# pangeo-data/scikit-downscale

Measured on AMD Instinct MI355X. Metric: grid-cells downscaled/sec (fit+predict), 40yr daily series, higher is better.
Workload: dtype f64; 1 GPU; BcsdTemperature quantile mapping, 100000 cells x 14600 steps per GPU (BASELINE configs[1]); cells_per_gpu=100000, total_cells=100000, groups=12, device= (gfx950:sramecc+:xnack-)

## Files before the change

scikit-downscale_amd/csrc/sd_bcsd_fx.hip:

```cpp
#include "sd_bcsd_rs.h"
#include "sd_wave.h"
#include "sd_wsort.h"

#ifdef SD_PHASE_MARKS
#define SDPH(name) asm volatile("; SDPHASE " name)
#else
#define SDPH(name)
#endif

namespace sdfx {

using namespace sdw;

#ifdef SD_DEV
constexpr int kTraceWgs = 256, kTraceSlots = 16, kTraceStride = 449;
__device__ long long sd_fx_trace[kTraceWgs * kTraceSlots];
#define SDT(slot)                                                                                              \
    do {                                                                                                       \
        if (traced) tstamp[slot] = (long long)__builtin_amdgcn_s_memtime();                                    \
    } while (0)
#else
#define SDT(slot)
#endif
using sdrs::Params;
// ... 570 lines not shown
                double v[K];
#pragma unroll
                for (int i = 0; i < K; ++i) v[i] = ob[i];
                double s = 0.0;
                if constexpr (FULL) {
#pragma unroll
                    for (int i = 0; i < K; ++i) s += v[i];
                    s = K * lane < n ? s : 0.0;
                } else {
#pragma unroll
                    for (int i = 0; i < K; ++i) s += K * lane + i < n ? v[i] : 0.0;
                }
                yc = wave_sum_f64(s) / (double)n;
                make_keys<K, false, FULL>(v, n, lane, ky);
            }
            SDT(10);
            SDPH("y_sort");
            if (!(abl & 2)) sdws::wave_sort<K>(ky, lane, (n + K - 1) / K);
            SDT(11);
            SDPH("y_fix");
            if (!(abl & 8)) redo_y = (fix_equal_q<K>(ky, rowb, lane) & kUnsorted) != 0 && cell_live;
            SDPH("y_gather");
            if constexpr (FULL) {
                const unsigned tm = K * lane < n ? kTagMask : 0u;
#pragma unroll
                for (int i = 0; i < K; ++i) t[i] = lds_f64(rowb + 8u * (ky[i] & tm));
            } else {
#pragma unroll
                for (int i = 0; i < K; ++i) t[i] = lds_f64(rowb + 8u * (K * lane + i < n ? (ky[i] & kTagMask) : (unsigned)(RS - 1)));
            }
            if (!IDENT) {
                wave_fence();
#pragma unroll
                for (int i = 0; i < K; ++i) lds_store_f64(K * lane + i < n ? rowb + 8u * (unsigned)(K * lane + i) : spare, t[i]);
            }
        }
    } else {
        SD_LANE();
        if (cell_ok) {
            yc = p->y_climo[seg];
            const double* src = p->ys + c * p->Tf + begf;
            for (int i = lane; i < n; i += kWave) row[i] = src[i];
        }
        wave_fence();
        if (IDENT) {
            const double* srow = row + (K * lane < n ? K * lane : 0);
#pragma unroll
            for (int i = 0; i < K; ++i) t[i] = srow[i];
        }
    }

    SDT(12);
    SDPH("map_scatter");
    int to[NR];
    {
        SD_LANE();
        if (!IDENT) {
            wave_fence();
            double slo = 0.0, ilo = 0.0, shi = 0.0, ihi = 0.0;
            if (m > n && n > 0) {
                const int e = n < p->n_endpoints ? n : p->n_endpoints;
                const double dn = pp_denom(n);
                ols_line(row, 0, e, dn, &slo, &ilo);
                ols_line(row, n - e, e, dn, &shi, &ihi);
            }
            const double nan = __longlong_as_double(0x7ff8000000000000ll);
            const int r0 = K * lane < m ? K * lane : 0;
            const int32_t* qi = p->qidx + begp + r0;
            const double* qv = p->qval + begp + r0;
#pragma unroll
            for (int i = 0; i < K; ++i) {
                const bool in = r0 + i < m;
                const int idx = in ? qi[i] : -3;
                const double w = in ? qv[i] : 0.0;
                double v;
                if (idx >= 0) {
                    const double y0 = row[idx];
                    const double y1 = row[idx + 1 < n ? idx + 1 : idx];
                    v = w == 0.0 ? y0 : y0 + w * (y1 - y0);
                } else if (idx == -1) {
                    v = w * slo + ilo;
                } else if (idx == -2) {
                    v = w * shi + ihi;
                } else {
                    v = nan;
                }
                t[i] = v;
                if ((i + 1) % CH == 0) __builtin_amdgcn_sched_barrier(0);
            }
        }
        wave_fence();
        const bool has = K * lane < m;
        if constexpr (FULL) {
            if (has) {
#pragma unroll
                for (int i = 0; i < K; ++i) lds_store_f64(rowb + 8u * (ku[i] & kTagMask), t[i]);
            }
        } else {
#pragma unroll
            for (int i = 0; i < K; ++i) lds_store_f64(K * lane + i < m ? rowb + 8u * (ku[i] & kTagMask) : spare, t[i]);
        }
        wave_fence();
        SDPH("restore");
        if (kEarlyRows) rows_load<NR, FULL>(p->ord_p + begp, m, to);
        double* ob = row + L::own(has ? lane : 0);
        double q[K];
#pragma unroll
        for (int i = 0; i < K; ++i) q[i] = ob[i];
        const double ycr = p->return_anoms ? yc : 0.0;
        if constexpr (FULL) {
            if (has) {
#pragma unroll
                for (int i = 0; i < K; ++i) ob[i] = (shift[i] + q[i]) - ycr;
            }
        } else {
#pragma unroll
            for (int i = 0; i < K; ++i) {
                const double res = (shift[i] + q[i]) - ycr;
                lds_store_f64(K * lane + i < m ? rowb + 8u * (unsigned)(L::own(lane) + i) : spare, res);
            }
        }
    }
    SDPH("store");
    SDT(13);
    redo_flag[wave] = redo_y ? 1 : 0;
    __syncthreads();
    SDT(14);
    any_redo = 0;
#pragma unroll
    for (int w = 0; w < kW; ++w) any_redo |= redo_flag[w];
    if (any_redo) {
        if (threadIdx.x == 0) {
            const int slot = atomicAdd(p->work_count, 1);
            if (slot < p->work_cap) p->worklist[slot] = tile_id * p->G + g;
        }
        return;
    }
    const bool vec_o = (p->ld_out % 2 == 0) && ((reinterpret_cast<uintptr_t>(p->out) & 15) == 0);
        if (!kEarlyRows) rows_load<NR, FULL>(p->ord_p + begp, m, to);
    if (!(abl & 16)) store_tile_ti<K, FULL>(p->out, p->ld_out, to, m, c0, p->C, vec_o, tile, RS);
#ifdef SD_DEV
    SDT(15);
    if (traced && threadIdx.x == 0) {
#pragma unroll
        for (int i = 0; i < kTraceSlots; ++i) sd_fx_trace[(blockIdx.x / kTraceStride) * kTraceSlots + i] = tstamp[i];
    }
#endif
#undef SD_LANE
}

namespace tmj {
constexpr int kChunkStride = 1024 + 8;
constexpr int kBlock = 20;
__host__ __device__ constexpr int chunks_of(int n) { return n / kBlock + 16; }
__device__ __forceinline__ int tail_chunk(int l) { return (l & 7) + 8 * (l >> 5); }
__device__ __forceinline__ int tail_slot(int l) { return (l >> 3) & 3; }
__device__ __forceinline__ int row_of_slot(int Q, int S, int nl, int n) {
    int r;
    if (Q < nl) {
        r = kBlock * Q + S;
    } else {
        const int t = Q - nl;
        const int l = (t & 7) + 8 * (S & 3) + 32 * (t >> 3);
        r = l < nl ? kBlock * l + 16 + (S >> 2) : n - 1;
    }
    return r < n ? r : n - 1;
}
__device__ __forceinline__ unsigned tag_off(unsigned tag) { return (tag << 6) + ((tag >> 4) << 3); }

template <int NREG>
struct RowIdx {
    int v[NREG];
};
template <int NREG>
__device__ __forceinline__ RowIdx<NREG> rows_of_wave(const int32_t* __restrict__ ord, int n, int q0, int wave, int lane) {
    RowIdx<NREG> t;
    const int nl = n / kBlock;
#pragma unroll
    for (int j = 0; j < NREG; ++j) {
        const int e = 64 * j + lane;
        t.v[j] = ord[row_of_slot(q0 + wave + kW * (e >> 4), e & 15, nl, n)];
    }
    return t;
}
template <int NREG>
__device__ __forceinline__ void rows_ready(RowIdx<NREG>& t) {
#pragma unroll
    for (int j = 0; j < NREG; ++j) asm volatile("" : "+v"(t.v[j]));
}
template <int NREG>
__device__ __forceinline__ int row_of_request(const RowIdx<NREG>& rows, int k, int lane) {
    return __builtin_amdgcn_ds_bpermute(4 * (16 * (k & 3) + (lane >> 2)), rows.v[k >> 2]);
}
template <int NK, int NREG>
__device__ __forceinline__ void dma_chunks(const double* __restrict__ src, int64_t ld, const RowIdx<NREG>& rows, int q0, int q1,
                                           int64_t c0, unsigned tile_b, int wave, int lane) {
    static_assert(NK <= 4 * NREG, "row registers");
    const char* colp = reinterpret_cast<const char*>(src + c0) + 16 * (lane & 3);
#pragma unroll
    for (int k = 0; k < NK; ++k) {
        const int q = q0 + wave + kW * k;
        if (q < q1) {
            const int ti = row_of_request(rows, k, lane);
            const char* g = colp + (uint64_t)(uint32_t)ti * (uint64_t)(uint32_t)((uint32_t)ld * 8u);
            const int dst = __builtin_amdgcn_readfirstlane((int)(tile_b + (unsigned)q * (unsigned)kChunkStride));
            unsigned keep;
            asm volatile("s_mov_b32 %0, m0\n\ts_mov_b32 m0, %2\n\ts_nop 0\n\tglobal_load_lds_dwordx4 %1, off\n\ts_mov_b32 m0, %0"
                         : "=&s"(keep)
                         : "v"(g), "s"(dst)
                         : "memory");
        }
    }
}
__device__ __forceinline__ void dma_wait_all() { asm volatile("s_waitcnt vmcnt(0)" ::: "memory"); }

struct Col {
    unsigned mainb, tailb, prevb;
    __device__ __forceinline__ unsigned at(int idx) const {
        return idx < 0 ? prevb + (unsigned)(256 * (idx + 4)) : idx < 16 ? mainb + (unsigned)(64 * idx)
             : idx < 20 ? tailb + (unsigned)(256 * (idx - 16)) : mainb + (unsigned)(kChunkStride + 64 * (idx - 20));
    }
    __device__ __forceinline__ double get(int idx) const {
        if (idx < 0) return reinterpret_cast<lds_cdouble_t*>((uintptr_t)prevb)[32 * (idx + 4)];
        if (idx < 16) return reinterpret_cast<lds_cdouble_t*>((uintptr_t)mainb)[8 * idx];
        if (idx < 20) return reinterpret_cast<lds_cdouble_t*>((uintptr_t)tailb)[32 * (idx - 16)];
        return reinterpret_cast<lds_cdouble_t*>((uintptr_t)mainb)[kChunkStride / 8 + 8 * (idx - 20)];
    }
    __device__ __forceinline__ void put(int idx, double x) const {
        if (idx < 16) reinterpret_cast<lds_double_t*>((uintptr_t)mainb)[8 * idx] = x;
        else reinterpret_cast<lds_double_t*>((uintptr_t)tailb)[32 * (idx - 16)] = x;
    }
};
__device__ __forceinline__ Col col_of(unsigned tile_b, int col, int bl, int nl) {
    const unsigned cb = tile_b + 8u * (unsigned)col;
    const int lp = (bl - 1) & 63;
    Col c;
    c.mainb = cb + (unsigned)bl * (unsigned)kChunkStride;
    c.tailb = cb + (unsigned)(nl + tail_chunk(bl)) * (unsigned)kChunkStride + 64u * (unsigned)tail_slot(bl);
    c.prevb = cb + (unsigned)(nl + tail_chunk(lp)) * (unsigned)kChunkStride + 64u * (unsigned)tail_slot(lp);
    return c;
}
struct Tags {
    unsigned main0, tail0;
    __device__ __forceinline__ unsigned of(int i) const { return i < 16 ? main0 + (unsigned)i : tail0 + (unsigned)(4 * (i - 16)); }
};
__device__ __forceinline__ Tags tags_of(int lane, int nl) {
    return Tags{16u * (unsigned)lane, 16u * (unsigned)(nl + tail_chunk(lane)) + (unsigned)tail_slot(lane)};
}

template <int K, class GetU>
__device__ __forceinline__ void keys_u2(const GetU& u_of, double lo, double hi, int m, int lane, const Tags& tg, unsigned (&key)[K], unsigned (&u2)[K]) {
    const double sc = (double)(kQD - 2u) / (hi - lo);
    const double off = -lo * sc + 1.0;
    const unsigned tag0 = (unsigned)(K * lane);
    const unsigned pad0 = ((kQD + 1u + tag0) << kTagBits) | tag0;
    const bool lane_in = K * lane < m;
#pragma unroll
    for (int i = 0; i < K; ++i) {
        const double t = __builtin_fma(u_of(i), sc, off) + 2097152.0;
        const unsigned w0 = (unsigned)__double2loint(t), w1 = (unsigned)__double2hiint(t);
        unsigned q = __builtin_amdgcn_alignbit(w1, w0, 31) & 0x1fffffu;
        q = q < kQD ? q : kQD;
        const unsigned dk = (q << kTagBits) | tg.of(i);
        const unsigned pk = pad0 + (unsigned)i * ((1u << kTagBits) + 1u);
        key[i] = lane_in ? dk : pk;
        u2[i] = w0;
    }
}
template <int K>
__device__ __forceinline__ void keys_pos(const double (&v)[K], int m, int lane, const Tags& tg, unsigned (&key)[K]) {
    double lo = __builtin_inf(), hi = -__builtin_inf();
#pragma unroll
    for (int i = 0; i < K; ++i) {
        lo = vmin(lo, v[i]);
        hi = vmax(hi, v[i]);
    }
    lo = wave_min_f64(lo);
    hi = wave_max_f64(hi);
    const double sc = (double)kQD / (hi - lo);
    const double off = -lo * sc;
    const unsigned tag0 = (unsigned)(K * lane);
    const unsigned pad0 = ((kQD + 1u + tag0) << kTagBits) | tag0;
    const bool lane_in = K * lane < m;
#pragma unroll
    for (int i = 0; i < K; ++i) {
        unsigned q = (unsigned)__builtin_fma(v[i], sc, off);
        q = q < kQD ? q : kQD;
        const unsigned dk = (q << kTagBits) | tg.of(i);
        const unsigned pk = pad0 + (unsigned)i * ((1u << kTagBits) + 1u);
        key[i] = lane_in ? dk : pk;
    }
}

template <int K, class Cmp>
__device__ __forceinline__ int fix_equal_q_by(unsigned (&k)[K], int lane, const Cmp& cmp) {
    constexpr unsigned kQ = 1u << kTagBits;
    bool tie = false;
#pragma unroll 1
    for (int pass = 0; pass < 6; ++pass) {
        bool swapped = false;
        const unsigned knext = from_next_lane(k[0], 0xffffffffu);
        const bool eqx = (k[K - 1] ^ knext) < kQ;
        const unsigned long long bx = __ballot(eqx);
        if (bx != 0ull) {
            bool gt, eq;
            cmp(k[K - 1] & kTagMask, knext & kTagMask, &gt, &eq);
            const bool sw = eqx && gt;
            tie |= eqx && eq;
            const unsigned d = sw ? (k[K - 1] ^ knext) : 0u;
            k[K - 1] ^= d;
            k[0] ^= from_prev_lane(d, 0u);
            swapped |= sw;
        }
        unsigned long long prev = 0ull, b0 = 0ull, multi = 0ull;
#pragma unroll
        for (int i = 0; i + 1 < K; ++i) {
            const bool e = (k[i] ^ k[i + 1]) < kQ;
            const unsigned long long b = __ballot(e);
            multi |= b & prev;
            if (i == 0) b0 = b;
            prev = b;
            if (b != 0ull) {
                bool gt, eq;
                cmp(k[i] & kTagMask, k[i + 1] & kTagMask, &gt, &eq);
                const bool sw = e && gt;
                tie |= e && eq;
                const unsigned d = sw ? (k[i] ^ k[i + 1]) : 0u;
                k[i] ^= d;
                k[i + 1] ^= d;
                swapped |= sw;
            }
        }
        multi |= (bx & prev) | ((bx << 1) & b0);
        if (multi == 0ull || !__any(swapped)) return __any(tie) ? kTie : 0;
    }
    return kUnsorted;
}
}

__host__ __device__ constexpr int fd_u2_stride(int nmax) { return 16 * tmj::chunks_of(nmax); }
__host__ __device__ constexpr int fd_late_chunks(int rsu) { return (kW * 4 * rsu + tmj::kChunkStride - 1) / tmj::kChunkStride; }
inline size_t fd_lds_bytes(int nmax) { return (size_t)kHeadDoubles * sizeof(double) + (size_t)tmj::chunks_of(nmax) * tmj::kChunkStride; }

template <int K, bool EARLY>
__global__ void __launch_bounds__(kThreads, 4) bcsd_fd_kernel(const Params) {
    extern __shared__ __attribute__((aligned(16))) char smem_raw[];
    ParamsPtr p = (ParamsPtr)__builtin_amdgcn_kernarg_segment_ptr();
    constexpr int NR = K / 2;
    constexpr int CH = K >= 20 ? K / 4 : K >= 14 ? K / 2 : K;
    constexpr int NKX = 10;
    static_assert(K == tmj::kBlock && K % CH == 0, "the chunk layout is that of 20 rows per lane");
#ifdef SD_DEV
    const int abl = p->dev_flags;
#else
    constexpr int abl = 0;
#endif
    double* const scratch = reinterpret_cast<double*>(smem_raw);
    int* const bad_cell = reinterpret_cast<int*>(scratch + 64 + 16);
    int* const redo_flag = bad_cell + kW;
    const unsigned tile_b = lds_addr(smem_raw) + (unsigned)(kHeadDoubles * sizeof(double));
    if (threadIdx.x >= 32 && threadIdx.x < 32 + kW) bad_cell[threadIdx.x - 32] = 0;
#ifdef SD_DEV
    const bool traced = (abl & 0x800) != 0 && blockIdx.x % kTraceStride == 7 && blockIdx.x / kTraceStride < (unsigned)kTraceWgs;
    long long tstamp[kTraceSlots] = {};
    SDT(0);
#endif
    int64_t tile_id;
    int g;
    xcd_tile_of_block(blockIdx.x, p->ntiles, &tile_id, &g);
    if (p->gmask != 0ull) g = nth_set_bit(p->gmask, g);
    if (tile_id >= p->ntiles || g < 0 || g >= p->G) return;

    const int64_t c0 = tile_id * kW;
    const int wave = __builtin_amdgcn_readfirstlane(tid_now() / kWave);
#define SD_LANE() const int lane = tid_now() % kWave
    const int64_t c = c0 + wave;
    const bool cell_ok = c < p->C;
    const int begf = p->off_f[g];
    const int m = p->off_f[g + 1] - begf;
    const int begp = p->off_p[g];
    if (m == 0) return;
    const int nl = m / K;
    const int nch = tmj::chunks_of(m);
    const int RSU = p->RS;
    const int nlate = fd_late_chunks(RSU) < nch ? fd_late_chunks(RSU) : nch;
    const bool cell_live = cell_ok && p->status_fit[cell_ok ? c : 0] == 0;
    const int64_t cfetch = c0 + kW <= p->C ? c0 : p->C - kW;
    const int cshift = (int)(c0 - cfetch);
    const int col = wave + cshift < kW ? wave + cshift : wave + cshift - kW;
    __syncthreads();

    SDPH("x_tiles");
    double xc = 0.0;
    tmj::RowIdx<EARLY ? 2 : 3> ry_late;
    tmj::RowIdx<2> ry_early;
    {
        SD_LANE();
        tmj::RowIdx<3> rp = tmj::rows_of_wave<3>(p->ord_p + begp, m, 0, wave, lane);
        TileRegs<NR> xh;
        int tf[NR];
        rows_load<NR, true>(p->ord_f + begf, m, tf);
        tmj::rows_ready(rp);
#pragma unroll
        for (int k = 0; k < NR; ++k) asm volatile("" : "+v"(tf[k]));
        if (!(abl & 64)) tmj::dma_chunks<NKX, 3>(p->Xp, p->ld_p, rp, 0, nch, cfetch, tile_b, wave, lane);
        if (!(abl & 4)) {
            const int cp = lane & 3;
            const double* src = p->X + (c0 + 2 * cp + 1 < p->C ? c0 + 2 * cp : c0);
#pragma unroll
            for (int k = 0; k < NR; ++k) {
                const double2 v = *reinterpret_cast<const double2*>(row_of(src, tf[k], p->ld));
                xh.v0[k] = v.x;
                xh.v1[k] = v.y;
            }
        }
        if (!(abl & 4)) tile_reduce_partials<NR, true>(xh, m, c0, p->C, scratch, p->status_fit, wave, lane, bad_cell);
        SDT(1);
        tmj::dma_wait_all();
    }
    __syncthreads();
    SDT(2);
    {
        double tot = 0.0;
#pragma unroll
        for (int w = 0; w < kW; ++w) tot += scratch[w * kW + wave];
        xc = tot / (double)m;
    }

    SDPH("rolling");
    double shift[K];
    unsigned ku[K];
    bool redo = false;
    {
        SD_LANE();
        const bool has = K * lane < m;
        const int bl = has ? lane : 0;
        const bool first_lane = bl == 0, last_lane = K * (bl + 1) == m;
        const tmj::Col cz = tmj::col_of(tile_b, col, bl, nl);
        double ulo = __builtin_inf(), uhi = -__builtin_inf();
        bool bad = false;
#pragma unroll
        for (int cbeg = 0; cbeg < K; cbeg += CH) {
            double w[CH + 8];
#pragma unroll
            for (int t = 0; t < CH + 8; ++t) {
                const int idx = cbeg - 4 + t;
                const double x = cz.get(idx);
                w[t] = idx < 0 ? (first_lane ? 0.0 : x) : idx >= K ? (last_lane ? 0.0 : x) : x;
            }
#pragma unroll
            for (int ii = 0; ii < CH; ++ii) {
                double s = 0.0;
#pragma unroll
                for (int d = 0; d < 9; ++d) s += w[ii + d];
                const int i = cbeg + ii;
                constexpr double kRc[10] = {0.0, 1.0, 0.5, 1.0 / 3.0, 0.25, 0.2, 1.0 / 6.0, 1.0 / 7.0, 0.125, 1.0 / 9.0};
                double cd = 9.0, rc = kRc[9];
                if (i < 4) {
                    cd = first_lane ? (double)(5 + i) : cd;
                    rc = first_lane ? kRc[5 + i] : rc;
                }
                if (i >= K - 4) {
                    cd = last_lane ? (double)(K + 4 - i) : cd;
                    rc = last_lane ? kRc[K + 4 - i] : rc;
                }
                const double q = s * rc;
                const double mean = __builtin_fma(__builtin_fma(-cd, q, s), rc, q);
                const double sh = mean - xc;
                shift[i] = sh;
                bad |= nonfinite64(w[ii + 4]);
                const double ui = (w[ii + 4] - sh) + 0.0;
                ulo = vmin(ulo, ui);
                uhi = vmax(uhi, ui);
            }
            __builtin_amdgcn_sched_barrier(0);
        }
        if (__any(bad && has)) {
            if (lane == 0) {
                if (cell_ok) atomicOr(&p->status_p[c], SDI_NONFINITE);
                bad_cell[wave] = 1;
            }
        }
        SDT(3);
        ry_late = tmj::rows_of_wave<EARLY ? 2 : 3>(p->ord_f + begf, m, 0, wave, lane);
        if (EARLY) ry_early = tmj::rows_of_wave<2>(p->ord_f + begf, m, nlate, wave, lane);
        SDPH("u_keys");
        unsigned u2[K];
        {
            ulo = wave_min_f64(ulo);
            uhi = wave_max_f64(uhi);
            const auto u_of = [&](int i) { return (cz.get(i) - shift[i]) + 0.0; };
            tmj::keys_u2<K>(u_of, ulo, uhi, m, lane, tmj::tags_of(lane, nl), ku, u2);
        }
        tmj::rows_ready(ry_late);
        unsigned ub;
        if constexpr (EARLY) {
            tmj::rows_ready(ry_early);
            __syncthreads();
            if (!(abl & 32)) tmj::dma_chunks<5, 2>(p->y, p->ld, ry_early, nlate, nch, cfetch, tile_b, wave, lane);
            ub = tile_b + 4u * (unsigned)(col * RSU);
        } else {
            wave_fence();
            ub = 0u;
        }
        if (!EARLY) {
            if (has) {
                const tmj::Col cw = tmj::col_of(tile_b, col, lane, nl);
#pragma unroll
                for (int i = 0; i < K; ++i) *reinterpret_cast<__attribute__((address_space(3))) unsigned*>((uintptr_t)cw.at(i)) = u2[i];
            }
        } else if (has) {
            const tmj::Tags tg = tmj::tags_of(lane, nl);
            typedef unsigned __attribute__((ext_vector_type(4))) u32x4;
            __attribute__((address_space(3))) u32x4* um = reinterpret_cast<__attribute__((address_space(3))) u32x4*>((uintptr_t)(ub + 4u * tg.main0));
#pragma unroll
            for (int i = 0; i < 16; i += 4) um[i / 4] = u32x4{u2[i], u2[i + 1], u2[i + 2], u2[i + 3]};
            __attribute__((address_space(3))) unsigned* ut = reinterpret_cast<__attribute__((address_space(3))) unsigned*>((uintptr_t)(ub + 4u * tg.tail0));
#pragma unroll
            for (int i = 16; i < K; ++i) ut[4 * (i - 16)] = u2[i];
        }
        wave_fence();
        SDT(4);
        SDPH("u_sort");
        if (!(abl & 1)) sdws::wave_sort<K>(ku, lane, (m + K - 1) / K);
        SDT(5);
        SDPH("u_fix");
        const unsigned colb_u = tile_b + 8u * (unsigned)col;
        const auto cmp_u2 = [ub, colb_u](unsigned ta, unsigned tb, bool* gt, bool* eq) {
            const unsigned a = lds_u32(EARLY ? ub + 4u * ta : colb_u + tmj::tag_off(ta)), b = lds_u32(EARLY ? ub + 4u * tb : colb_u + tmj::tag_off(tb));
            *gt = a > b;
            *eq = a == b;
        };
        const bool tie = (abl & 8) ? false : tmj::fix_equal_q_by<K>(ku, lane, cmp_u2) != 0;
        redo = tie && cell_live && bad_cell[wave] == 0 && (abl & 0x7ff) == 0;
        SDT(6);
    }
    SDPH("vote");
    redo_flag[wave] = redo ? 1 : 0;
    __syncthreads();
    int any_redo = 0;
#pragma unroll
    for (int w = 0; w < kW; ++w) any_redo |= redo_flag[w];
    if (any_redo) {
        tmj::dma_wait_all();
        if (threadIdx.x == 0) {
            const int slot = atomicAdd(p->work_count, 1);
            if (slot < p->work_cap) p->worklist[slot] = tile_id * p->G + g;
        }
        return;
    }
    SDT(7);

    SDPH("y_tile");
    double yc = 0.0;
    double t[K];
    bool redo_y = false;
    {
        SD_LANE();
        if (!(abl & 32)) tmj::dma_chunks<EARLY ? 5 : NKX, EARLY ? 2 : 3>(p->y, p->ld, ry_late, 0, EARLY ? nlate : nch, cfetch, tile_b, wave, lane);
        SDT(8);
        tmj::dma_wait_all();
        __syncthreads();
        SDT(9);
        SDPH("y_keys");
        const bool has = K * lane < m;
        const int bl = has ? lane : 0;
        const tmj::Col cz = tmj::col_of(tile_b, col, bl, nl);
        const unsigned colb = tile_b + 8u * (unsigned)col;
        unsigned ky[K];
        {
            double v[K];
#pragma unroll
            for (int i = 0; i < K; ++i) v[i] = cz.get(i);
            double s = 0.0;
            bool bad = false;
#pragma unroll
            for (int i = 0; i < K; ++i) {
                s += v[i];
                bad |= nonfinite64(v[i]);
            }
            s = has ? s : 0.0;
            yc = wave_sum_f64(s) / (double)m;
            if (__any(bad && has) && lane == 0 && cell_ok) atomicOr(&p->status_fit[c], SDI_NONFINITE);
            tmj::keys_pos<K>(v, m, lane, tmj::tags_of(lane, nl), ky);
        }
        SDT(10);
        SDPH("y_sort");
        if (!(abl & 2)) sdws::wave_sort<K>(ky, lane, (m + K - 1) / K);
        SDT(11);
        SDPH("y_fix");
        const auto cmp_y = [colb](unsigned ta, unsigned tb, bool* gt, bool* eq) {
            const double a = lds_f64(colb + tmj::tag_off(ta)), b = lds_f64(colb + tmj::tag_off(tb));
            *gt = a > b;
            *eq = a == b;
        };
        if (!(abl & 8)) redo_y = (tmj::fix_equal_q_by<K>(ky, lane, cmp_y) & kUnsorted) != 0 && cell_live;
        SDPH("y_gather");
        {
            const unsigned tm = has ? kTagMask : 0u;
#pragma unroll
            for (int i = 0; i < K; ++i) t[i] = lds_f64(colb + tmj::tag_off(ky[i] & tm));
        }
        SDT(12);
        SDPH("map_scatter");
        wave_fence();
        if (has) {
#pragma unroll
            for (int i = 0; i < K; ++i) lds_store_f64(colb + tmj::tag_off(ku[i] & kTagMask), t[i]);
        }
        wave_fence();
        SDPH("restore");
        double q[K];
#pragma unroll
        for (int i = 0; i < K; ++i) q[i] = cz.get(i);
        const double ycr = p->return_anoms ? yc : 0.0;
        if (has) {
#pragma unroll
            for (int i = 0; i < K; ++i) cz.put(i, (shift[i] + q[i]) - ycr);
        }
    }
    SDPH("store");
    SDT(13);
    redo_flag[wave] = redo_y ? 1 : 0;
    tmj::RowIdx<3> ro = tmj::rows_of_wave<3>(p->ord_p + begp, m, 0, wave, tid_now() % kWave);
    __syncthreads();
    tmj::rows_ready(ro);
    SDT(14);
    any_redo = 0;
#pragma unroll
    for (int w = 0; w < kW; ++w) any_redo |= redo_flag[w];
    if (any_redo) {
        if (threadIdx.x == 0) {
            const int slot = atomicAdd(p->work_count, 1);
            if (slot < p->work_cap) p->worklist[slot] = tile_id * p->G + g;
        }
        return;
    }
    if (!(abl & 16)) {
        SD_LANE();
        const int pair = 2 * (lane & 3);
        const bool keep = pair >= cshift;
        char* colp = reinterpret_cast<char*>(p->out + cfetch) + 16 * (lane & 3);
#pragma unroll
        for (int k = 0; k < NKX; ++k) {
            const int qc = wave + kW * k;
            const int S = lane >> 2;
            const bool row_in = qc < nl ? K * qc + S < m : (((qc - nl) & 7) + 8 * (S & 3) + 32 * ((qc - nl) >> 3)) < nl;
            const int ti = tmj::row_of_request(ro, k, lane);
            if (qc < nch && row_in && keep) {
                typedef double __attribute__((ext_vector_type(2))) f64x2;
                const f64x2 v = *reinterpret_cast<__attribute__((address_space(3))) const f64x2*>((uintptr_t)(tile_b + (unsigned)qc * (unsigned)tmj::kChunkStride + 16u * (unsigned)lane));
                *reinterpret_cast<f64x2*>(colp + (uint64_t)(uint32_t)ti * (uint64_t)(uint32_t)((uint32_t)p->ld_out * 8u)) = v;
            }
        }
    }
#ifdef SD_DEV
    SDT(15);
    if (traced && threadIdx.x == 0) {
#pragma unroll
        for (int i = 0; i < kTraceSlots; ++i) sd_fx_trace[(blockIdx.x / kTraceStride) * kTraceSlots + i] = tstamp[i];
    }
#endif
#undef SD_LANE
}

template <int K, bool IDENT, bool FULL>
__device__ __forceinline__ void fxp_segment(ParamsPtr p, int64_t tile_id, int g, char* smem_raw) {
    static_assert(!FULL || IDENT, "FULL launches serve groups of equal fit / predict length");
    constexpr int NR = K / 2;
    constexpr int CH = K >= 20 ? K / 4 : K >= 14 ? K / 2 : K;
    using L = Lay<K>;
    double* const scratch = reinterpret_cast<double*>(smem_raw);
    int* const bad_cell = reinterpret_cast<int*>(scratch + 64 + 16);
    int* const redo_flag = bad_cell + kW;
    double* const tile = scratch + kHeadDoubles;
    const int RS = p->RS;
    if (threadIdx.x >= 32 && threadIdx.x < 32 + kW) bad_cell[threadIdx.x - 32] = 0;

    const int64_t c0 = tile_id * kW;
    const int wave = __builtin_amdgcn_readfirstlane(tid_now() / kWave);
#define SD_LANE() const int lane = tid_now() % kWave
    const int64_t c = c0 + wave;
    const bool cell_ok = c < p->C;
    double* const row = tile + wave * RS;
    const unsigned rowb = lds_addr(row);
    const int64_t seg = c * p->G + g;
    const int begf = p->off_f[g];
    const int n = p->off_f[g + 1] - begf;
    const int begp = p->off_p[g];
    const int m = p->off_p[g + 1] - begp;
    if (m == 0) return;
    const bool vec_f = (p->ld % 2 == 0) && ((reinterpret_cast<uintptr_t>(p->y) & 15) == 0) &&
                       (p->X == nullptr || (reinterpret_cast<uintptr_t>(p->X) & 15) == 0);
    const bool vec_p = (p->ld_p % 2 == 0) && ((reinterpret_cast<uintptr_t>(p->Xp) & 15) == 0);
    const bool cell_live = cell_ok && p->status_fit[cell_ok ? c : 0] == 0;
    const unsigned spare = rowb + 8u * (unsigned)(RS - 1);
    __syncthreads();

    {
        TileRegs<NR> xf;
        int tp[NR];
        rows_load<NR, FULL>(p->ord_p + begp, m, tp);
        if (!p->from_state && p->X != nullptr && n > 0) {
            TileRegs<NR> xh;
            int tf[NR];
            rows_load<NR, FULL>(p->ord_f + begf, n, tf);
            tile_issue_ti<NR>(p->X, p->ld, tf, c0, p->C, vec_f, xh);
            tile_issue_ti<NR>(p->Xp, p->ld_p, tp, c0, p->C, vec_p, xf);
            tile_check_finite<NR>(xh, n, c0, p->C, p->status_fit, bad_cell);
        } else {
            tile_issue_ti<NR>(p->Xp, p->ld_p, tp, c0, p->C, vec_p, xf);
        }
        tile_commit_sw<NR, K, FULL>(xf, m, c0, p->C, tile, RS, p->status_p, bad_cell);
    }
    __syncthreads();

    unsigned ku[K];
    int n0 = 0;
    bool redo = false;
    TileRegs<NR> yt;
    {
        SD_LANE();
        const double* ob = row + L::own(K * lane < m ? lane : 0);
        double v[K];
#pragma unroll
        for (int i = 0; i < K; ++i) v[i] = ob[i];
        if constexpr (FULL) {
            const bool has = K * lane < m;
#pragma unroll
            for (int i = 0; i < K; ++i) n0 += __popcll(__ballot(has && v[i] == 0.0));
        } else {
#pragma unroll
            for (int i = 0; i < K; ++i) n0 += __popcll(__ballot(K * lane + i < m && v[i] == 0.0));
        }
        const double lo = make_keys<K, true, FULL>(v, m, lane, ku);
        if (!p->from_state && n > 0) {
            int ty[NR];
            rows_load<NR, FULL>(p->ord_f + begf, n, ty);
            tile_issue_ti<NR>(p->y, p->ld, ty, c0, p->C, vec_f, yt);
        }
        sdws::wave_sort<K>(ku, lane, (m + K - 1) / K);
        const bool tie = fix_equal_q<K, true>(ku, rowb, lane) != 0;
        redo = (tie || lo < 0.0) && cell_live && bad_cell[wave] == 0;
    }
    redo_flag[wave] = redo ? 1 : 0;
    __syncthreads();
    int any_redo = 0;
#pragma unroll
    for (int w = 0; w < kW; ++w) any_redo |= redo_flag[w];
    if (any_redo) {
        if (threadIdx.x == 0) {
            const int slot = atomicAdd(p->work_count, 1);
            if (slot < p->work_cap) p->worklist[slot] = tile_id * p->G + g;
        }
        return;
    }

    double yc = 0.0;
    bool redo_y = false;
    if (!p->from_state) {
        if (n > 0) {
            SD_LANE();
            tile_commit_sw<NR, K, FULL>(yt, n, c0, p->C, tile, RS, p->status_fit, nullptr);
            __syncthreads();
            unsigned ky[K];
            {
                const double* ob = row + L::own(K * lane < n ? lane : 0);
                double v[K];
#pragma unroll
                for (int i = 0; i < K; ++i) v[i] = ob[i];
                double s = 0.0;
                if constexpr (FULL) {
#pragma unroll
                    for (int i = 0; i < K; ++i) s += v[i];
                    s = K * lane < n ? s : 0.0;
                } else {
#pragma unroll
                    for (int i = 0; i < K; ++i) s += K * lane + i < n ? v[i] : 0.0;
                }
                yc = wave_sum_f64(s) / (double)n;
                if (lane == 0 && cell_ok && p->return_anoms && yc <= 0.0) atomicOr(&p->status_fit[c], SDI_BAD_CLIMO);
                const double lo = make_keys<K, true, FULL>(v, n, lane, ky);
                redo_y = lo < 0.0 && cell_live;
            }
            sdws::wave_sort<K>(ky, lane, (n + K - 1) / K);
            redo_y = (redo_y || (fix_equal_q<K, true>(ky, rowb, lane) & kUnsorted) != 0) && cell_live;
            double t[K];
            if constexpr (FULL) {
                const unsigned tm = K * lane < n ? kTagMask : 0u;
#pragma unroll
                for (int i = 0; i < K; ++i) t[i] = lds_f64(rowb + 8u * (ky[i] & tm));
            } else {
#pragma unroll
                for (int i = 0; i < K; ++i) t[i] = lds_f64(rowb + 8u * (K * lane + i < n ? (ky[i] & kTagMask) : (unsigned)(RS - 1)));
            }
            wave_fence();
            if constexpr (FULL) {
                if (K * lane < n) {
#pragma unroll
                    for (int i = 0; i < K; ++i) lds_store_f64(rowb + 8u * (unsigned)(K * lane + i), t[i]);
// ... 306 lines not shown
            const double lo = make_keys_plain<KC>(vc, nw_y, lane, ky);
            sdws::wave_sort<KC>(ky, lane, (nw_y + KC - 1) / KC);
            redo_y = (lo < 0.0 || (fix_equal_q<KC>(ky, rowb, lane) & kUnsorted) != 0) && cell_live;
            double t[KC];
            const unsigned tm = KC * lane < nw_y ? kTagMask : 0u;
#pragma unroll
            for (int i = 0; i < KC; ++i) t[i] = lds_f64(rowb + 8u * (ky[i] & tm));
            wave_fence();
            if (KC * lane < nw_y) {
#pragma unroll
                for (int i = 0; i < KC; ++i) lds_store_f64(KC * lane + i < nw_y ? rowb + 8u * (unsigned)(KC * lane + i) : spare, t[i]);
            }
            wave_fence();
        }
    }

    int to[NR];
    {
        SD_LANE();
        const int n0_x = m - nw_x;
        auto ys = [&](int r) -> double {
            const double w = row[r >= n0_y ? r - n0_y : 0];
            return r >= n0_y ? w : 0.0;
        };
        double t[KC];
#pragma unroll
        for (int i = 0; i < KC; ++i) {
            const int rw = KC * lane + i;
            t[i] = ys(rw < nw_x ? n0_x + rw : 0);
        }
        const double val0 = ys(n0_x > 0 ? n0_x - 1 : 0);
        wave_fence();
        if (KC * lane < nw_x) {
#pragma unroll
            for (int i = 0; i < KC; ++i) lds_store_f64(KC * lane + i < nw_x ? rowb + 8u * (kx[i] & kTagMask) : spare, t[i]);
        }
        wave_fence();
        double q[K];
        {
            const double* cp = row + base_x;
            int pos = 0;
#pragma unroll
            for (int i = 0; i < K; ++i) {
                const bool wet = ((zm_x >> i) & 1u) == 0u;
                const double wv = cp[wet ? pos : 0];
                q[i] = wet ? wv : val0;
                pos += wet ? 1 : 0;
            }
        }
        wave_fence();
        const bool has = K * lane < m;
        rows_load<NR, FULL>(p->ord_p + begp, m, to);
        if (has) {
            double* ob = row + L::own(lane);
            const double rc = 1.0 / yc;
#pragma unroll
            for (int i = 0; i < K; ++i) {
                double res = q[i];
                if (p->return_anoms) {
                    const double a = q[i] * rc;
                    res = __builtin_fma(__builtin_fma(-yc, a, q[i]), rc, a);
                    res = __builtin_isfinite(res) ? res : q[i] / yc;
                }
                ob[i] = res;
            }
        }
    }
    redo_flag[wave] = (redo_y ? 1 : 0) | (many_y ? 2 : 0);
    __syncthreads();
    any_redo = 0;
#pragma unroll
    for (int w = 0; w < kW; ++w) any_redo |= redo_flag[w];
    if (any_redo) {
        if (threadIdx.x == 0) {
            if (any_redo & 1) {
                const int slot = atomicAdd(p->work_count, 1);
                if (slot < p->work_cap) p->worklist[slot] = tile_id * p->G + g;
            } else {
                const int slot = atomicAdd(p->work_count2, 1);
                if (slot < p->work_cap) p->worklist2[slot] = tile_id * p->G + g;
            }
        }
        return;
    }
    const bool vec_o = (p->ld_out % 2 == 0) && ((reinterpret_cast<uintptr_t>(p->out) & 15) == 0);
    store_tile_ti<K, FULL>(p->out, p->ld_out, to, m, c0, p->C, vec_o, tile, RS);
#undef SD_LANE
}

template <int K, bool IDENT, bool FULL>
int launch_one(sd_ctx* ctx, const Params& p, size_t lds) {
    const int64_t tx = (p.ntiles + 7) / 8;
    const int64_t nblocks = 8 * tx * (p.gmask ? __builtin_popcountll(p.gmask) : p.G);
    SD_CHECK_ARG(nblocks < ((int64_t)1 << 31), "grid too large");
    if (p.kind == SD_BCSD_TAS) {
        SD_HIP(hipFuncSetAttribute(reinterpret_cast<const void*>(&bcsd_fx_kernel<K, IDENT, FULL>), hipFuncAttributeMaxDynamicSharedMemorySize,
                                   (int)lds));
        SD_LAUNCH(ctx, FULL ? "bcsd_fx_kernel_full" : "bcsd_fx_kernel", (bcsd_fx_kernel<K, IDENT, FULL>), dim3((unsigned)nblocks),
                  dim3(kThreads), lds, p);
    } else {
        SD_HIP(hipFuncSetAttribute(reinterpret_cast<const void*>(&bcsd_fxp_kernel<K, IDENT, FULL>), hipFuncAttributeMaxDynamicSharedMemorySize,
                                   (int)lds));
        SD_LAUNCH(ctx, FULL ? "bcsd_fxp_kernel_full" : "bcsd_fxp_kernel", (bcsd_fxp_kernel<K, IDENT, FULL>), dim3((unsigned)nblocks),
                  dim3(kThreads), lds, p);
    }
    return SD_OK;
}

template <int K, bool IDENT>
int launch_ki(sd_ctx* ctx, Params p, int nmax, const int* group_len) {
    p.RS = row_slots<K>(nmax);
    const size_t lds = ((size_t)kW * p.RS + kHeadDoubles) * sizeof(double);
    if (lds > ctx->lds_max) return sd_set_error(SD_ERR_UNSUPPORTED, "segment of %d samples needs %zu bytes of LDS", nmax, lds);
    unsigned long long full = 0ull, rest = 0ull;
#ifndef SD_FX_NOFULL
    if (IDENT && group_len != nullptr && p.G <= 64 && sd_dev_env("SD_FX_NOFULL") == nullptr) {
        for (int g = 0; g < p.G; ++g) {
            const bool f = group_len[g] % K == 0 && group_len[g] >= full_min_len<K>();
            (f ? full : rest) |= 1ull << g;
        }
    }
#endif
#ifndef SD_FX_NOCOMPACT
    if constexpr (IDENT && compact_width<K>() != 0) {
        if (p.kind == SD_BCSD_PR && !p.from_state && p.work_count2 != nullptr && p.G <= 64 && group_len != nullptr &&
            sd_dev_env("SD_FX_NOCOMPACT") == nullptr) {
            constexpr int KC = compact_width<K>();
            Params q = p;
            if ((full | rest) == 0ull) rest = p.G == 64 ? ~0ull : (1ull << p.G) - 1ull;
            if (full != 0ull) {
                q.gmask = full;
                const int64_t nb = 8 * ((p.ntiles + 7) / 8) * __builtin_popcountll(full);
                SD_CHECK_ARG(nb < ((int64_t)1 << 31), "grid too large");
                SD_HIP(hipFuncSetAttribute(reinterpret_cast<const void*>(&bcsd_fxc_kernel<K, KC, true>), hipFuncAttributeMaxDynamicSharedMemorySize, (int)lds));
                SD_LAUNCH(ctx, "bcsd_fxc_kernel_full", (bcsd_fxc_kernel<K, KC, true>), dim3((unsigned)nb), dim3(kThreads), lds, q);
            }
            if (rest != 0ull) {
                q.gmask = rest;
                const int64_t nb = 8 * ((p.ntiles + 7) / 8) * __builtin_popcountll(rest);
                SD_CHECK_ARG(nb < ((int64_t)1 << 31), "grid too large");
                SD_HIP(hipFuncSetAttribute(reinterpret_cast<const void*>(&bcsd_fxc_kernel<K, KC, false>), hipFuncAttributeMaxDynamicSharedMemorySize, (int)lds));
                SD_LAUNCH(ctx, "bcsd_fxc_kernel", (bcsd_fxc_kernel<K, KC, false>), dim3((unsigned)nb), dim3(kThreads), lds, q);
            }
            Params r = p;
            r.use_worklist = 2;
            SD_HIP(hipFuncSetAttribute(reinterpret_cast<const void*>(&bcsd_fxp_kernel<K, IDENT, false>), hipFuncAttributeMaxDynamicSharedMemorySize, (int)lds));
            SD_LAUNCH(ctx, "bcsd_fxp_kernel_list", (bcsd_fxp_kernel<K, IDENT, false>), dim3((unsigned)(2 * (ctx->cu_count > 0 ? ctx->cu_count : 256))),
                      dim3(kThreads), lds, r);
            return SD_OK;
        }
    }
#endif
    if constexpr (IDENT && K == 20) {
        int nfull = 0;
        for (int g = 0; g < p.G && group_len != nullptr && p.G <= 64; ++g)
            if ((full >> g) & 1ull) nfull = group_len[g] > nfull ? group_len[g] : nfull;
        const auto al16 = [](const void* q) { return (reinterpret_cast<uintptr_t>(q) & 15) == 0; };
        const size_t lds_fd = fd_lds_bytes(nfull);
        const bool ok = full != 0ull && p.kind == SD_BCSD_TAS && !p.from_state && p.X != nullptr && p.C >= kW && p.C % 2 == 0 && p.ld % 2 == 0 &&
                        p.ld_p % 2 == 0 && p.ld_out % 2 == 0 && al16(p.X) && al16(p.y) && al16(p.Xp) && al16(p.out) && 2 * lds_fd <= ctx->lds_max &&
                        nfull % 20 == 0 && nfull > 640 && tmj::chunks_of(nfull) <= 80 && fd_late_chunks(fd_u2_stride(nfull)) <= 40 &&
                        tmj::chunks_of(nfull) - fd_late_chunks(fd_u2_stride(nfull)) <= 40 && sd_dev_env("SD_FX_NODMA") == nullptr;
        if (ok) {
            Params q = p;
            q.gmask = full;
            q.RS = fd_u2_stride(nfull);
            const int64_t nb = 8 * ((p.ntiles + 7) / 8) * __builtin_popcountll(full);
            SD_CHECK_ARG(nb < ((int64_t)1 << 31), "grid too large");
            if (sd_dev_env("SD_FD_LATE") != nullptr) {
                SD_HIP(hipFuncSetAttribute(reinterpret_cast<const void*>(&bcsd_fd_kernel<K, false>), hipFuncAttributeMaxDynamicSharedMemorySize, (int)lds_fd));
                SD_LAUNCH(ctx, "bcsd_fd_kernel", (bcsd_fd_kernel<K, false>), dim3((unsigned)nb), dim3(kThreads), lds_fd, q);
            } else {
                SD_HIP(hipFuncSetAttribute(reinterpret_cast<const void*>(&bcsd_fd_kernel<K, true>), hipFuncAttributeMaxDynamicSharedMemorySize, (int)lds_fd));
                SD_LAUNCH(ctx, "bcsd_fd_kernel", (bcsd_fd_kernel<K, true>), dim3((unsigned)nb), dim3(kThreads), lds_fd, q);
            }
            if (rest == 0ull) return SD_OK;
            q = p;
            q.gmask = rest;
            return launch_one<K, IDENT, false>(ctx, q, lds);
        }
    }
    if (IDENT && full != 0ull) {
        Params q = p;
        q.gmask = full;
        SD_TRY((launch_one<K, IDENT, IDENT>(ctx, q, lds)));
        if (rest == 0ull) return SD_OK;
        q.gmask = rest;
        return launch_one<K, IDENT, false>(ctx, q, lds);
    }
    return launch_one<K, IDENT, false>(ctx, p, lds);
}

template <int K>
int launch_k(sd_ctx* ctx, const Params& p, int nmax, const int* gl) {
    return p.identity ? launch_ki<K, true>(ctx, p, nmax, gl) : launch_ki<K, false>(ctx, p, nmax, gl);
}

int launch_width(sd_ctx* ctx, const Params& p, int nmax, const int* gl) {
#ifdef SD_FX_ONLY_K
    if (true) return launch_k<SD_FX_ONLY_K>(ctx, p, nmax, gl);
#else
    if (nmax <= 64 * 4) return launch_k<4>(ctx, p, nmax, gl);
    if (nmax <= 64 * 8) return launch_k<8>(ctx, p, nmax, gl);
    if (nmax <= 64 * 12) return launch_k<12>(ctx, p, nmax, gl);
    if (nmax <= 64 * 16) return launch_k<16>(ctx, p, nmax, gl);
    if (nmax <= 64 * 20) return launch_k<20>(ctx, p, nmax, gl);
    if (nmax <= 64 * 24) return launch_k<24>(ctx, p, nmax, gl);
#endif
    return sd_set_error(SD_ERR_UNSUPPORTED, "segment of %d samples exceeds the fused register-sort path", nmax);
}

}

bool sd_bcsd_fx_supported(int nmax) { return nmax >= 1 && nmax <= 64 * 24; }

int sd_bcsd_fx_launch(sd_ctx* ctx, const sdrs::Params& p, int nmax, const int* group_len) {
    sdrs::Params q = p;
    q.gmask = 0ull;
    q.use_worklist = 0;
    if (q.n_endpoints <= 0) q.n_endpoints = 10;
    SD_TRY(sdfx::launch_width(ctx, q, nmax, group_len));
#ifdef SD_DEV
    if (const char* path = sd_dev_env("SD_FX_TRACE")) {
        SD_HIP(hipStreamSynchronize(ctx->stream));
        std::vector<long long> h((size_t)sdfx::kTraceWgs * sdfx::kTraceSlots);
        SD_HIP(hipMemcpyFromSymbol(h.data(), HIP_SYMBOL(sdfx::sd_fx_trace), h.size() * sizeof(long long)));
        if (FILE* f = fopen(path, "wb")) {
            fwrite(h.data(), sizeof(long long), h.size(), f);
            fclose(f);
        }
    }
#endif
    return SD_OK;
}
```

Measured before the change: 6.672 million cells/s.

## Extend fused DMA kernel to ragged-length groups via RAG template path

Adds a RAG template variant of the fused-DMA BCSD kernel so that groups whose length is not a multiple of 20 (the 'rest' groups) can use the fast LDS-tiled path instead of the generic fallback kernel. Chunk/lane counts now round up, per-element masking is applied to padding keys, window sums and min/max, and a reciprocal table replaces constant divisors for ragged edges. The host launcher now classifies full and rest groups separately and launches the ragged kernel when its size limits fit. This adds per-element predicates and a table lookup in the inner loops for ragged groups.

```diff
diff --git a/scikit-downscale_amd/csrc/sd_bcsd_fx.hip b/scikit-downscale_amd/csrc/sd_bcsd_fx.hip
--- a/scikit-downscale_amd/csrc/sd_bcsd_fx.hip
+++ b/scikit-downscale_amd/csrc/sd_bcsd_fx.hip
@@ -746,7 +746,8 @@
 namespace tmj {
 constexpr int kChunkStride = 1024 + 8;
 constexpr int kBlock = 20;
-__host__ __device__ constexpr int chunks_of(int n) { return n / kBlock + 16; }
+__host__ __device__ constexpr int lanes_of(int n) { return (n + kBlock - 1) / kBlock; }
+__host__ __device__ constexpr int chunks_of(int n) { return lanes_of(n) + 16; }
 __device__ __forceinline__ int tail_chunk(int l) { return (l & 7) + 8 * (l >> 5); }
 __device__ __forceinline__ int tail_slot(int l) { return (l >> 3) & 3; }
 __device__ __forceinline__ int row_of_slot(int Q, int S, int nl, int n) {
@@ -769,7 +770,7 @@
 template <int NREG>
 __device__ __forceinline__ RowIdx<NREG> rows_of_wave(const int32_t* __restrict__ ord, int n, int q0, int wave, int lane) {
     RowIdx<NREG> t;
-    const int nl = n / kBlock;
+    const int nl = lanes_of(n);
 #pragma unroll
     for (int j = 0; j < NREG; ++j) {
         const int e = 64 * j + lane;
@@ -842,7 +843,7 @@
     return Tags{16u * (unsigned)lane, 16u * (unsigned)(nl + tail_chunk(lane)) + (unsigned)tail_slot(lane)};
 }
 
-template <int K, class GetU>
+template <int K, bool RAG, class GetU>
 __device__ __forceinline__ void keys_u2(const GetU& u_of, double lo, double hi, int m, int lane, const Tags& tg, unsigned (&key)[K], unsigned (&u2)[K]) {
     const double sc = (double)(kQD - 2u) / (hi - lo);
     const double off = -lo * sc + 1.0;
@@ -857,11 +858,11 @@
         q = q < kQD ? q : kQD;
         const unsigned dk = (q << kTagBits) | tg.of(i);
         const unsigned pk = pad0 + (unsigned)i * ((1u << kTagBits) + 1u);
-        key[i] = lane_in ? dk : pk;
+        key[i] = (RAG ? K * lane + i < m : lane_in) ? dk : pk;
         u2[i] = w0;
     }
 }
-template <int K>
+template <int K, bool RAG>
 __device__ __forceinline__ void keys_pos(const double (&v)[K], int m, int lane, const Tags& tg, unsigned (&key)[K]) {
     double lo = __builtin_inf(), hi = -__builtin_inf();
 #pragma unroll
@@ -882,7 +883,7 @@
         q = q < kQD ? q : kQD;
         const unsigned dk = (q << kTagBits) | tg.of(i);
         const unsigned pk = pad0 + (unsigned)i * ((1u << kTagBits) + 1u);
-        key[i] = lane_in ? dk : pk;
+        key[i] = (RAG ? K * lane + i < m : lane_in) ? dk : pk;
     }
 }
 
@@ -936,7 +937,7 @@
 __host__ __device__ constexpr int fd_late_chunks(int rsu) { return (kW * 4 * rsu + tmj::kChunkStride - 1) / tmj::kChunkStride; }
 inline size_t fd_lds_bytes(int nmax) { return (size_t)kHeadDoubles * sizeof(double) + (size_t)tmj::chunks_of(nmax) * tmj::kChunkStride; }
 
-template <int K, bool EARLY>
+template <int K, bool EARLY, bool RAG>
 __global__ void __launch_bounds__(kThreads, 4) bcsd_fd_kernel(const Params) {
     extern __shared__ __attribute__((aligned(16))) char smem_raw[];
     ParamsPtr p = (ParamsPtr)__builtin_amdgcn_kernarg_segment_ptr();
@@ -950,9 +951,11 @@
     constexpr int abl = 0;
 #endif
     double* const scratch = reinterpret_cast<double*>(smem_raw);
+    double* const rcp = scratch + 64;
     int* const bad_cell = reinterpret_cast<int*>(scratch + 64 + 16);
     int* const redo_flag = bad_cell + kW;
     const unsigned tile_b = lds_addr(smem_raw) + (unsigned)(kHeadDoubles * sizeof(double));
+    if (RAG) fill_rcp_table(rcp);
     if (threadIdx.x >= 32 && threadIdx.x < 32 + kW) bad_cell[threadIdx.x - 32] = 0;
 #ifdef SD_DEV
     const bool traced = (abl & 0x800) != 0 && blockIdx.x % kTraceStride == 7 && blockIdx.x / kTraceStride < (unsigned)kTraceWgs;
@@ -974,7 +977,7 @@
     const int m = p->off_f[g + 1] - begf;
     const int begp = p->off_p[g];
     if (m == 0) return;
-    const int nl = m / K;
+    const int nl = RAG ? tmj::lanes_of(m) : m / K;
     const int nch = tmj::chunks_of(m);
     const int RSU = p->RS;
     const int nlate = fd_late_chunks(RSU) < nch ? fd_late_chunks(RSU) : nch;
@@ -993,7 +996,7 @@
         tmj::RowIdx<3> rp = tmj::rows_of_wave<3>(p->ord_p + begp, m, 0, wave, lane);
         TileRegs<NR> xh;
         int tf[NR];
-        rows_load<NR, true>(p->ord_f + begf, m, tf);
+        rows_load<NR, !RAG>(p->ord_f + begf, m, tf);
         tmj::rows_ready(rp);
 #pragma unroll
         for (int k = 0; k < NR; ++k) asm volatile("" : "+v"(tf[k]));
@@ -1008,7 +1011,7 @@
                 xh.v1[k] = v.y;
             }
         }
-        if (!(abl & 4)) tile_reduce_partials<NR, true>(xh, m, c0, p->C, scratch, p->status_fit, wave, lane, bad_cell);
+        if (!(abl & 4)) tile_reduce_partials<NR, !RAG>(xh, m, c0, p->C, scratch, p->status_fit, wave, lane, bad_cell);
         SDT(1);
         tmj::dma_wait_all();
     }
@@ -1030,6 +1033,7 @@
         const bool has = K * lane < m;
         const int bl = has ? lane : 0;
         const bool first_lane = bl == 0, last_lane = K * (bl + 1) == m;
+        const int rl = m - K * bl;
         const tmj::Col cz = tmj::col_of(tile_b, col, bl, nl);
         double ulo = __builtin_inf(), uhi = -__builtin_inf();
         bool bad = false;
@@ -1040,7 +1044,8 @@
             for (int t = 0; t < CH + 8; ++t) {
                 const int idx = cbeg - 4 + t;
                 const double x = cz.get(idx);
-                w[t] = idx < 0 ? (first_lane ? 0.0 : x) : idx >= K ? (last_lane ? 0.0 : x) : x;
+                if (RAG) w[t] = idx < 0 ? (first_lane ? 0.0 : x) : idx >= rl ? 0.0 : x;
+                else w[t] = idx < 0 ? (first_lane ? 0.0 : x) : idx >= K ? (last_lane ? 0.0 : x) : x;
             }
 #pragma unroll
             for (int ii = 0; ii < CH; ++ii) {
@@ -1050,22 +1055,31 @@
                 const int i = cbeg + ii;
                 constexpr double kRc[10] = {0.0, 1.0, 0.5, 1.0 / 3.0, 0.25, 0.2, 1.0 / 6.0, 1.0 / 7.0, 0.125, 1.0 / 9.0};
                 double cd = 9.0, rc = kRc[9];
-                if (i < 4) {
-                    cd = first_lane ? (double)(5 + i) : cd;
-                    rc = first_lane ? kRc[5 + i] : rc;
-                }
-                if (i >= K - 4) {
-                    cd = last_lane ? (double)(K + 4 - i) : cd;
-                    rc = last_lane ? kRc[K + 4 - i] : rc;
+                if constexpr (RAG) {
+                    int cnt = rl + 4 - i;
+                    cnt = cnt < 9 ? (cnt > 1 ? cnt : 1) : 9;
+                    if (i < 4) cnt = first_lane ? 5 + i : cnt;
+                    cd = (double)cnt;
+                    rc = rcp[cnt];
+                } else {
+                    if (i < 4) {
+                        cd = first_lane ? (double)(5 + i) : cd;
+                        rc = first_lane ? kRc[5 + i] : rc;
+                    }
+                    if (i >= K - 4) {
+                        cd = last_lane ? (double)(K + 4 - i) : cd;
+                        rc = last_lane ? kRc[K + 4 - i] : rc;
+                    }
                 }
                 const double q = s * rc;
                 const double mean = __builtin_fma(__builtin_fma(-cd, q, s), rc, q);
                 const double sh = mean - xc;
                 shift[i] = sh;
                 bad |= nonfinite64(w[ii + 4]);
-                const double ui = (w[ii + 4] - sh) + 0.0;
-                ulo = vmin(ulo, ui);
-                uhi = vmax(uhi, ui);
+                const double ui = w[ii + 4] - sh;
+                const bool in = !RAG || i < rl;
+                ulo = vmin(ulo, in ? ui : ulo);
+                uhi = vmax(uhi, in ? ui : uhi);
             }
             __builtin_amdgcn_sched_barrier(0);
         }
@@ -1083,8 +1097,8 @@
         {
             ulo = wave_min_f64(ulo);
             uhi = wave_max_f64(uhi);
-            const auto u_of = [&](int i) { return (cz.get(i) - shift[i]) + 0.0; };
-            tmj::keys_u2<K>(u_of, ulo, uhi, m, lane, tmj::tags_of(lane, nl), ku, u2);
+            const auto u_of = [&](int i) { return cz.get(i) - shift[i]; };
+            tmj::keys_u2<K, RAG>(u_of, ulo, uhi, m, lane, tmj::tags_of(lane, nl), ku, u2);
         }
         tmj::rows_ready(ry_late);
         unsigned ub;
@@ -1168,15 +1182,16 @@
             for (int i = 0; i < K; ++i) v[i] = cz.get(i);
             double s = 0.0;
             bool bad = false;
+            const int rl = m - K * bl;
 #pragma unroll
             for (int i = 0; i < K; ++i) {
-                s += v[i];
+                s += !RAG || i < rl ? v[i] : 0.0;
                 bad |= nonfinite64(v[i]);
             }
             s = has ? s : 0.0;
             yc = wave_sum_f64(s) / (double)m;
             if (__any(bad && has) && lane == 0 && cell_ok) atomicOr(&p->status_fit[c], SDI_NONFINITE);
-            tmj::keys_pos<K>(v, m, lane, tmj::tags_of(lane, nl), ky);
+            tmj::keys_pos<K, RAG>(v, m, lane, tmj::tags_of(lane, nl), ky);
         }
         SDT(10);
         SDPH("y_sort");
@@ -1199,8 +1214,9 @@
         SDPH("map_scatter");
         wave_fence();
         if (has) {
-#pragma unroll
-            for (int i = 0; i < K; ++i) lds_store_f64(colb + tmj::tag_off(ku[i] & kTagMask), t[i]);
+            const tmj::Tags tg = tmj::tags_of(lane, nl);
+#pragma unroll
+            for (int i = 0; i < K; ++i) lds_store_f64(colb + tmj::tag_off(!RAG || K * lane + i < m ? ku[i] & kTagMask : tg.of(i)), t[i]);
         }
         wave_fence();
         SDPH("restore");
@@ -1239,7 +1255,8 @@
         for (int k = 0; k < NKX; ++k) {
             const int qc = wave + kW * k;
             const int S = lane >> 2;
-            const bool row_in = qc < nl ? K * qc + S < m : (((qc - nl) & 7) + 8 * (S & 3) + 32 * ((qc - nl) >> 3)) < nl;
+            const int lt = ((qc - nl) & 7) + 8 * (S & 3) + 32 * ((qc - nl) >> 3);
+            const bool row_in = qc < nl ? K * qc + S < m : RAG ? K * lt + 16 + (S >> 2) < m : lt < nl;
             const int ti = tmj::row_of_request(ro, k, lane);
             if (qc < nch && row_in && keep) {
                 typedef double __attribute__((ext_vector_type(2))) f64x2;
@@ -1852,30 +1869,48 @@
     }
 #endif
     if constexpr (IDENT && K == 20) {
-        int nfull = 0;
-        for (int g = 0; g < p.G && group_len != nullptr && p.G <= 64; ++g)
-            if ((full >> g) & 1ull) nfull = group_len[g] > nfull ? group_len[g] : nfull;
+        int nmx[2] = {0, 0}, nmn[2] = {1 << 30, 1 << 30};
+        for (int g = 0; g < p.G && group_len != nullptr && p.G <= 64; ++g) {
+            const int s = ((full >> g) & 1ull) ? 0 : ((rest >> g) & 1ull) ? 1 : -1;
+            if (s < 0) continue;
+            nmx[s] = group_len[g] > nmx[s] ? group_len[g] : nmx[s];
+            nmn[s] = group_len[g] < nmn[s] ? group_len[g] : nmn[s];
+        }
         const auto al16 = [](const void* q) { return (reinterpret_cast<uintptr_t>(q) & 15) == 0; };
-        const size_t lds_fd = fd_lds_bytes(nfull);
-        const bool ok = full != 0ull && p.kind == SD_BCSD_TAS && !p.from_state && p.X != nullptr && p.C >= kW && p.C % 2 == 0 && p.ld % 2 == 0 &&
-                        p.ld_p % 2 == 0 && p.ld_out % 2 == 0 && al16(p.X) && al16(p.y) && al16(p.Xp) && al16(p.out) && 2 * lds_fd <= ctx->lds_max &&
-                        nfull % 20 == 0 && nfull > 640 && tmj::chunks_of(nfull) <= 80 && fd_late_chunks(fd_u2_stride(nfull)) <= 40 &&
-                        tmj::chunks_of(nfull) - fd_late_chunks(fd_u2_stride(nfull)) <= 40 && sd_dev_env("SD_FX_NODMA") == nullptr;
-        if (ok) {
+        const bool fields = p.kind == SD_BCSD_TAS && !p.from_state && p.X != nullptr && p.C >= kW && p.C % 2 == 0 && p.ld % 2 == 0 &&
+                            p.ld_p % 2 == 0 && p.ld_out % 2 == 0 && al16(p.X) && al16(p.y) && al16(p.Xp) && al16(p.out) &&
+                            sd_dev_env("SD_FX_NODMA") == nullptr;
+        const auto fits = [&](int s) {
+            const int n = nmx[s];
+            return nmn[s] > 640 && tmj::chunks_of(n) <= 80 && fd_late_chunks(fd_u2_stride(n)) <= 40 &&
+                   tmj::chunks_of(n) - fd_late_chunks(fd_u2_stride(n)) <= 40 && 2 * fd_lds_bytes(n) <= ctx->lds_max;
+        };
+        const bool late = sd_dev_env("SD_FD_LATE") != nullptr;
+        const auto launch_fd = [&](unsigned long long mask, int s, auto kern, const char* name) -> int {
             Params q = p;
-            q.gmask = full;
-            q.RS = fd_u2_stride(nfull);
-            const int64_t nb = 8 * ((p.ntiles + 7) / 8) * __builtin_popcountll(full);
+            q.gmask = mask;
+            q.RS = fd_u2_stride(nmx[s]);
+            const size_t lds_fd = fd_lds_bytes(nmx[s]);
+            const int64_t nb = 8 * ((p.ntiles + 7) / 8) * __builtin_popcountll(mask);
             SD_CHECK_ARG(nb < ((int64_t)1 << 31), "grid too large");
-            if (sd_dev_env("SD_FD_LATE") != nullptr) {
-                SD_HIP(hipFuncSetAttribute(reinterpret_cast<const void*>(&bcsd_fd_kernel<K, false>), hipFuncAttributeMaxDynamicSharedMemorySize, (int)lds_fd));
-                SD_LAUNCH(ctx, "bcsd_fd_kernel", (bcsd_fd_kernel<K, false>), dim3((unsigned)nb), dim3(kThreads), lds_fd, q);
-            } else {
-                SD_HIP(hipFuncSetAttribute(reinterpret_cast<const void*>(&bcsd_fd_kernel<K, true>), hipFuncAttributeMaxDynamicSharedMemorySize, (int)lds_fd));
-                SD_LAUNCH(ctx, "bcsd_fd_kernel", (bcsd_fd_kernel<K, true>), dim3((unsigned)nb), dim3(kThreads), lds_fd, q);
-            }
+            SD_HIP(hipFuncSetAttribute(reinterpret_cast<const void*>(kern), hipFuncAttributeMaxDynamicSharedMemorySize, (int)lds_fd));
+            SD_LAUNCH(ctx, name, kern, dim3((unsigned)nb), dim3(kThreads), lds_fd, q);
+            return SD_OK;
+        };
+        const bool fd_full = fields && full != 0ull && fits(0), fd_rest = fields && rest != 0ull && fits(1);
+        if (fd_full || fd_rest) {
+            if (fd_full) {
+                SD_TRY(late ? launch_fd(full, 0, &bcsd_fd_kernel<K, false, false>, "bcsd_fd_kernel")
+                            : launch_fd(full, 0, &bcsd_fd_kernel<K, true, false>, "bcsd_fd_kernel"));
+            } else if (full != 0ull) {
+                Params q = p;
+                q.gmask = full;
+                SD_TRY((launch_one<K, IDENT, IDENT>(ctx, q, lds)));
+            }
+            if (fd_rest) return late ? launch_fd(rest, 1, &bcsd_fd_kernel<K, false, true>, "bcsd_fd_kernel_ragged")
+                                     : launch_fd(rest, 1, &bcsd_fd_kernel<K, true, true>, "bcsd_fd_kernel_ragged");
             if (rest == 0ull) return SD_OK;
-            q = p;
+            Params q = p;
             q.gmask = rest;
             return launch_one<K, IDENT, false>(ctx, q, lds);
         }
```

Result: faster. 6.793 million cells/s, median of 6 (+1.8%).
